# G-U-N/Phased-Consistency-Model

Measured on NVIDIA H100. Metric: distillation steps/sec (SD1.5 PCM-LoRA, bs=8/GPU), higher is better.
Workload: dtype bf16

## Files before the change

pcm_b200/csrc/gemm_epilogue.cuh:

```cuda
#pragma once
#include "gemm_params.h"

namespace pcm {

static __device__ __noinline__ void gemm_epilogue_rows_generic(const GemmParams& p, const float* sb, int m0,
                                                               int n, int r0, int cg, float* ws) {
#pragma unroll 1
  for (int i = 0; i < 2; ++i) {
    const int rr = r0 + 32 * i;
    const int m = m0 + rr;
    if (m >= p.M) continue;
    const float* srow = sb + rr * 32;
    if (ws) {
      const float4 a0 = *reinterpret_cast<const float4*>(srow + ((2 * cg) ^ (rr & 7)) * 4);
      const float4 a1 = *reinterpret_cast<const float4*>(srow + ((2 * cg + 1) ^ (rr & 7)) * 4);
      const float f[8] = {a0.x, a0.y, a0.z, a0.w, a1.x, a1.y, a1.z, a1.w};
      float* wp = ws + static_cast<long long>(m) * p.N + n;
      if (n + 8 <= p.N && (p.N & 3) == 0) {
        *reinterpret_cast<float4*>(wp) = make_float4(f[0] * p.alpha, f[1] * p.alpha, f[2] * p.alpha, f[3] * p.alpha);
        *reinterpret_cast<float4*>(wp + 4) = make_float4(f[4] * p.alpha, f[5] * p.alpha, f[6] * p.alpha, f[7] * p.alpha);
      } else {
#pragma unroll
        for (int e = 0; e < 8; ++e)
          if (n + e < p.N) wp[e] = f[e] * p.alpha;
// ... 111 lines not shown
#pragma unroll
      for (int i = 0; i < 2; ++i) {
        if (!valid[i]) continue;
        const float4 a0 = lds128(ld_a0 + i * 4096);
        const float4 a1 = lds128(ld_a1 + i * 4096);
        float f[8] = {a0.x, a0.y, a0.z, a0.w, a1.x, a1.y, a1.z, a1.w};
        if (p.alpha != 1.0f) {
#pragma unroll
          for (int e = 0; e < 8; ++e) f[e] *= p.alpha;
        }
        f[0] += bia0.x; f[1] += bia0.y; f[2] += bia0.z; f[3] += bia0.w;
        f[4] += bia1.x; f[5] += bia1.y; f[6] += bia1.z; f[7] += bia1.w;
        if (has_rv) add_bf16x8(f, rrv[i]);
        if (has_res) add_bf16x8(f, rcur[i]);
        uint4 u;
        u.x = pack_bf16x2(f[0], f[1]);
        u.y = pack_bf16x2(f[2], f[3]);
        u.z = pack_bf16x2(f[4], f[5]);
        u.w = pack_bf16x2(f[6], f[7]);
        *reinterpret_cast<uint4*>(reinterpret_cast<bf16*>(p.out) + off[i] + n) = u;
      }
      if (has_res) {
#pragma unroll
        for (int i = 0; i < 2; ++i) rcur[i] = rnext[i];
        load_res(rnext, j + 2);
      }
    } else if (n < p.N) {
      gemm_epilogue_rows_generic(p, sb, m0, n, r0, cg, ws);
    }
    asm volatile("bar.sync %0, 128;" ::"r"(bar) : "memory");
  }
}

}
```

pcm_b200/csrc/gemm_params.h:

```cpp
#pragma once
#include <cuda.h>
#include "common.cuh"
#include "../../include/pcm_b200.h"

namespace pcm {

struct KEntry {
  int a_map, b_map, dw, dh, nchunks, a_c0, b_k0;
  unsigned short n_lo, n_hi;
  int m_hi;
  int kend;
};

struct alignas(64) GemmParams {
  CUtensorMap a_maps[PCM_MAX_ASRC];
  CUtensorMap b_maps[PCM_MAX_BSRC];
  KEntry prog[PCM_MAX_PROG];
  int num_prog, lin;
  int M, N;
  int geoW, geoHW;
  int block_n, tiles_m, tiles_n, num_kblocks, num_stages;
  void* out;
  const float* bias;
  const bf16* rowvec;
  const bf16* residual;
  long long osW, osH, osB, rowvec_ld;
  int epiW, epiHW;
  int out_fp32, round_bf16;
  float alpha;
  int act;
  int b_blocked;
  int dep_a_map;
  int filtered;
  int ksplit;
  float* ws;
};

constexpr int kATileBytes = 128 * 128;

}
```

pcm_b200/csrc/gemm_tc.cu:

```cuda
#include "common.cuh"
#include "wgmma.cuh"
#include "host_common.h"
#include "../../include/pcm_b200.h"
#include "gemm_params.h"
#include "gemm_epilogue.cuh"

namespace pcm {

constexpr int kGemmThreads = 384;
constexpr int kWgradThreads = 256;
constexpr int kMaxStages = 8;
constexpr int kStagingBytes = 2 * 64 * 32 * 4;
constexpr int kSmemLimit = 227 * 1024 - 512;

__device__ __forceinline__ int tile_kblocks(const GemmParams& p, int m0, int n0) {
  int nkb = 0;
  for (int e = 0; e < p.num_prog; ++e) {
    const KEntry en = p.prog[e];
    if ((en.n_hi == 0 || (n0 >= en.n_lo && n0 < en.n_hi)) && (en.m_hi == 0 || m0 < en.m_hi))
      nkb += en.nchunks;
  }
  return nkb;
}

__device__ __forceinline__ int chunk_ksteps(int kend, int c) {
  const int w = kend - 64 * c;
  return w >= 64 ? 4 : (w <= 16 ? 1 : (w + 15) >> 4);
}

template <int BN, bool NARROW>
__global__ void __launch_bounds__(kGemmThreads, 1)
pcm_gemm_kernel(const __grid_constant__ GemmParams p) {
  extern __shared__ uint8_t smem_raw[];
  uint8_t* smem = reinterpret_cast<uint8_t*>((reinterpret_cast<uintptr_t>(smem_raw) + 1023) &
                                             ~static_cast<uintptr_t>(1023));
  __shared__ __align__(8) uint64_t full_bar[kMaxStages];
  __shared__ __align__(8) uint64_t empty_bar[kMaxStages];
  __shared__ int stage_ksteps[NARROW ? kMaxStages : 1];

  const int wg = threadIdx.x >> 7;
  const int S = p.num_stages;
  constexpr uint32_t stage_bytes = kATileBytes + BN * 128;
  const int num_items = p.tiles_m * p.tiles_n * p.ksplit;
  const int kb_per = (p.num_kblocks + p.ksplit - 1) / p.ksplit;

  if (threadIdx.x == 0) {
    for (int i = 0; i < PCM_MAX_ASRC; ++i) tma_prefetch_desc(&p.a_maps[i]);
    for (int i = 0; i < PCM_MAX_BSRC; ++i) tma_prefetch_desc(&p.b_maps[i]);
    for (int i = 0; i < S; ++i) {
      mbar_init(&full_bar[i], 1);
      mbar_init(&empty_bar[i], 2);
    }
    fence_barrier_init();
  }
  __syncthreads();
  if (p.dep_a_map < 0) griddep_sync();
  else griddep_launch();

  if (wg == 0) {
    regs_dealloc<40>();
    if (threadIdx.x == 0) {
      int stage = 0;
      uint32_t phase = 0;
      bool dep_waited = p.dep_a_map < 0;
      for (int item = blockIdx.x; item < num_items; item += gridDim.x) {
        const int tile = item / p.ksplit, ks = item - tile * p.ksplit;
        const int kb0 = ks * kb_per, kb1 = min(p.num_kblocks, kb0 + kb_per);
        int tm = tile / p.tiles_n;
        const int tn = tile - tm * p.tiles_n;
        if (p.dep_a_map >= 0) tm = p.tiles_m - 1 - tm;
        const int m0 = tm * 128, n0 = tn * BN;
        int b0 = 0, h0 = 0;
        if (!p.lin) {
          b0 = m0 / p.geoHW;
          h0 = (m0 - b0 * p.geoHW) / p.geoW;
        }
        int kidx = 0;
        for (int e = 0; e < p.num_prog; ++e) {
          const KEntry en = p.prog[e];
          if (en.n_hi != 0 && (n0 < en.n_lo || n0 >= en.n_hi)) continue;
          if (en.m_hi != 0 && m0 >= en.m_hi) continue;
          if (kidx + en.nchunks <= kb0 || kidx >= kb1) {
            kidx += en.nchunks;
            continue;
          }
          if (!dep_waited && en.a_map == p.dep_a_map) {
            griddep_wait();
            dep_waited = true;
          }
          for (int c = 0; c < en.nchunks; ++c, ++kidx) {
            if (kidx < kb0 || kidx >= kb1) continue;
            mbar_wait(&empty_bar[stage], phase ^ 1);
            if constexpr (NARROW) stage_ksteps[stage] = chunk_ksteps(en.kend, c);
            mbar_arrive_expect_tx(&full_bar[stage], stage_bytes);
            uint8_t* sa = smem + stage * stage_bytes;
            uint8_t* sb = sa + kATileBytes;
            if (p.lin)
              tma_load_4d(sa, &p.a_maps[en.a_map], &full_bar[stage], en.a_c0 + c * 64, m0, 0, 0);
            else
              tma_load_4d(sa, &p.a_maps[en.a_map], &full_bar[stage], en.a_c0 + c * 64, en.dw,
                          h0 + en.dh, b0);
            if ((p.b_blocked >> en.b_map) & 1)
              tma_load_3d(sb, &p.b_maps[en.b_map], &full_bar[stage], 0, n0, (en.b_k0 >> 6) + c);
            else
              tma_load_2d(sb, &p.b_maps[en.b_map], &full_bar[stage], en.b_k0 + c * 64, n0);
            if (++stage == S) {
              stage = 0;
              phase ^= 1;
            }
          }
        }
      }
    }
  } else {
    regs_alloc<232>();
    const int cw = wg - 1;
    const int et = threadIdx.x & 127;
    float* sbuf = reinterpret_cast<float*>(smem + S * stage_bytes) + cw * (64 * 32);
    float acc[BN / 2];
    int stage = 0;
    uint32_t phase = 0;
    for (int item = blockIdx.x; item < num_items; item += gridDim.x) {
      const int tile = item / p.ksplit, ks = item - tile * p.ksplit;
      int tm = tile / p.tiles_n;
      const int tn = tile - tm * p.tiles_n;
      if (p.dep_a_map >= 0) tm = p.tiles_m - 1 - tm;
      const int n0 = tn * BN;
      const int nkb = p.filtered ? tile_kblocks(p, tm * 128, n0)
                                 : min(p.num_kblocks, (ks + 1) * kb_per) - ks * kb_per;
      if (nkb <= 0) {
#pragma unroll
        for (int i = 0; i < BN / 2; ++i) acc[i] = 0.f;
      }
      int prev_stage = -1;
      for (int kb = 0; kb < nkb; ++kb) {
        mbar_wait(&full_bar[stage], phase);
        const uint32_t a_addr = smem_u32(smem + stage * stage_bytes) + cw * (64 * 128);
        const uint32_t b_addr = smem_u32(smem + stage * stage_bytes) + kATileBytes;
        wgmma_fence();
        if constexpr (NARROW) {
          const int nk = stage_ksteps[stage];
#pragma unroll
          for (int k = 0; k < 4; ++k)
            if (k < nk)
              Wgmma<BN, 0, 0>::mma(acc, wgmma_desc_sw128(a_addr + k * 32, 16, 1024),
                                   wgmma_desc_sw128(b_addr + k * 32, 16, 1024), (kb | k) != 0 ? 1u : 0u);
        } else {
#pragma unroll
          for (int k = 0; k < 4; ++k)
            Wgmma<BN, 0, 0>::mma(acc, wgmma_desc_sw128(a_addr + k * 32, 16, 1024),
                                 wgmma_desc_sw128(b_addr + k * 32, 16, 1024), (kb | k) != 0 ? 1u : 0u);
        }
        wgmma_commit();
        wgmma_fence_acc(acc);
        wgmma_wait<1>();
        if (prev_stage >= 0 && et == 0) mbar_arrive(&empty_bar[prev_stage]);
        prev_stage = stage;
        if (++stage == S) {
          stage = 0;
          phase ^= 1;
        }
      }
      wgmma_wait<0>();
      wgmma_fence_acc(acc);
      if (prev_stage >= 0 && et == 0) mbar_arrive(&empty_bar[prev_stage]);
      float* ws = p.ws ? p.ws + static_cast<long long>(ks) * p.M * p.N : nullptr;
      gemm_epilogue_tile<BN>(p, tm * 128 + cw * 64, n0, acc, sbuf, et, 1 + cw, ws);
    }
  }
}

__global__ void splitk_finalize_kernel(const GemmParams p) {
  griddep_sync();
  const int nvec = (p.N + 7) >> 3;
  const long long total = static_cast<long long>(p.M) * nvec;
  const long long slice = static_cast<long long>(p.M) * p.N;
  const bool vec = (p.N & 7) == 0;
  for (long long v = blockIdx.x * static_cast<long long>(blockDim.x) + threadIdx.x; v < total;
       v += static_cast<long long>(gridDim.x) * blockDim.x) {
    const int m = static_cast<int>(v / nvec);
    const int n = static_cast<int>(v - static_cast<long long>(m) * nvec) * 8;
    const int b = m / p.epiHW;
    const int r = m - b * p.epiHW;
    const int h = r / p.epiW;
    const int w = r - h * p.epiW;
    const long long o = b * p.osB + h * p.osH + w * p.osW;
    float x[8];
    const float* wp = p.ws + static_cast<long long>(m) * p.N + n;
    if (vec) {
      float4 a0 = *reinterpret_cast<const float4*>(wp), a1 = *reinterpret_cast<const float4*>(wp + 4);
#pragma unroll 4
      for (int k = 1; k < p.ksplit; ++k) {
        const float4 b0 = *reinterpret_cast<const float4*>(wp + k * slice);
        const float4 b1 = *reinterpret_cast<const float4*>(wp + k * slice + 4);
        a0.x += b0.x; a0.y += b0.y; a0.z += b0.z; a0.w += b0.w;
        a1.x += b1.x; a1.y += b1.y; a1.z += b1.z; a1.w += b1.w;
      }
      x[0] = a0.x; x[1] = a0.y; x[2] = a0.z; x[3] = a0.w;
      x[4] = a1.x; x[5] = a1.y; x[6] = a1.z; x[7] = a1.w;
    } else {
// ... 169 lines not shown
        atomicExch(sem, blockIdx.z + 1 == gridDim.z ? 0 : static_cast<int>(blockIdx.z) + 1);
    }
  }
}

static int encode_asrc(CUtensorMap* map, const pcm_asrc& a, int lin, int geoW, int geoH,
                       int box_c = 64) {
  cuuint64_t dims[4];
  cuuint64_t strides[3];
  cuuint32_t box[4];
  cuuint32_t estr[4] = {1, 1, 1, 1};
  if (lin) {
    dims[0] = a.C; dims[1] = a.W; dims[2] = 1; dims[3] = 1;
    strides[0] = a.sW * 2;
    strides[1] = static_cast<cuuint64_t>(a.sW) * 2 * a.W;
    strides[2] = strides[1];
    box[0] = box_c; box[1] = 128; box[2] = 1; box[3] = 1;
  } else {
    dims[0] = a.C; dims[1] = a.W; dims[2] = a.H; dims[3] = a.B;
    strides[0] = a.sW * 2; strides[1] = a.sH * 2; strides[2] = a.sB * 2;
    const int bw = geoW;
    if (bw > 128 || 128 % bw != 0) return set_error("conv geometry: W must divide 128");
    int bh = 128 / bw;
    if (bh > geoH) bh = geoH;
    int bb = 128 / (bw * bh);
    if (bw * bh * bb != 128) return set_error("conv geometry: H*W must divide or be divisible by 128");
    box[0] = box_c; box[1] = bw; box[2] = bh; box[3] = bb;
  }
  return encode_tmap(map, a.ptr, 4, dims, strides, box, estr);
}

typedef void (*GemmKernel)(const GemmParams);
template <bool NARROW>
static GemmKernel gemm_kernel_for(int block_n) {
  switch (block_n) {
    case 32: return pcm_gemm_kernel<32, NARROW>;
    case 64: return pcm_gemm_kernel<64, NARROW>;
    case 96: return pcm_gemm_kernel<96, NARROW>;
    case 128: return pcm_gemm_kernel<128, NARROW>;
    case 160: return pcm_gemm_kernel<160, NARROW>;
    case 192: return pcm_gemm_kernel<192, NARROW>;
    case 224: return pcm_gemm_kernel<224, NARROW>;
    default: return pcm_gemm_kernel<256, NARROW>;
  }
}

static bool misaligned(const void* p, uintptr_t a) { return (reinterpret_cast<uintptr_t>(p) & (a - 1)) != 0; }

static bool gemm_ranged(const pcm_gemm_desc* d) {
  for (int e = 0; e < d->num_prog; ++e)
    if (d->prog[e].n_hi != 0) return true;
  return false;
}

static int gemm_ksplit(const pcm_gemm_desc* d) {
  if (d->ksplit <= 1 || d->splitk_ws == nullptr || gemm_ranged(d)) return 1;
  int nkb = 0;
  for (int e = 0; e < d->num_prog; ++e) nkb += d->prog[e].nchunks;
  if (nkb < 1) return 1;
  const int ks = d->ksplit < nkb ? d->ksplit : nkb;
  const int per = (nkb + ks - 1) / ks;
  return (nkb + per - 1) / per;
}

static int validate_gemm(const pcm_gemm_desc* d) {
  if (d->block_n < 32 || d->block_n > 256 || (d->block_n % 32) != 0)
    return set_error("pcm_gemm: block_n must be a multiple of 32 in [32, 256]");
  if (d->num_a < 1 || d->num_a > PCM_MAX_ASRC || d->num_b < 1 || d->num_b > PCM_MAX_BSRC ||
      d->num_prog < 1 || d->num_prog > PCM_MAX_PROG)
    return set_error("pcm_gemm: bad source / program counts");
  if (d->M < 1) return set_error("pcm_gemm: M must be >= 1");
  if (d->N < 1) return set_error("pcm_gemm: N must be >= 1");
  if (d->out == nullptr) return set_error("pcm_gemm: out is null");
  if (!d->lin && (d->geoW < 1 || d->geoH < 1)) return set_error("pcm_gemm: geoW and geoH must be >= 1 in conv mode");
  if (!d->lin && d->epiW < 1) return set_error("pcm_gemm: epiW must be >= 1 in conv mode");
  if (!d->lin && d->epiHW < 1) return set_error("pcm_gemm: epiHW must be >= 1 in conv mode");
  if (d->act != 0 && d->act != 1) return set_error("pcm_gemm: act must be 0 or 1");
  if (d->dep_a_src1 < 0 || d->dep_a_src1 > d->num_a) return set_error("pcm_gemm: bad dep_a_src1");
  if (d->ksplit > 1 && !gemm_ranged(d)) {
    if (d->splitk_ws == nullptr) return set_error("pcm_gemm: ksplit > 1 needs splitk_ws");
    if (misaligned(d->splitk_ws, 16)) return set_error("pcm_gemm: splitk_ws is not 16-byte aligned");
  }
  const bool wide = !d->out_fp32 && d->act == 0 && gemm_ksplit(d) == 1;
  const bool vec = wide && d->N >= 32;
  const bool vec_res = wide && d->residual != nullptr && d->N >= 8;
  if (misaligned(d->out, vec ? 16 : (d->out_fp32 ? 4 : 2)))
    return set_error(vec ? "pcm_gemm: out is not 16-byte aligned" : "pcm_gemm: out is not aligned to its element size");
  if (d->bias && misaligned(d->bias, vec ? 16 : 4))
    return set_error(vec ? "pcm_gemm: bias is not 16-byte aligned" : "pcm_gemm: bias is not 4-byte aligned");
  if (d->rowvec && misaligned(d->rowvec, vec ? 16 : 2))
    return set_error(vec ? "pcm_gemm: rowvec is not 16-byte aligned" : "pcm_gemm: rowvec is not 2-byte aligned");
  if (d->residual && misaligned(d->residual, vec_res ? 16 : 2))
    return set_error(vec_res ? "pcm_gemm: residual is not 16-byte aligned" : "pcm_gemm: residual is not 2-byte aligned");
  if (vec || vec_res) {
    if (d->osW % 8 != 0) return set_error("pcm_gemm: osW is not a multiple of 8");
    if (d->osH % 8 != 0) return set_error("pcm_gemm: osH is not a multiple of 8");
    if (d->osB % 8 != 0) return set_error("pcm_gemm: osB is not a multiple of 8");
  }
  if (vec && d->rowvec && d->rowvec_ld % 8 != 0) return set_error("pcm_gemm: rowvec_ld is not a multiple of 8");
  return 0;
}

static int validate_wgrad(const pcm_wgrad_desc* d) {
  if (d->M < 1) return set_error("pcm_wgrad: M must be >= 1");
  if (d->out == nullptr) return set_error("pcm_wgrad: out is null");
  if (d->os_row == 0) return set_error("pcm_wgrad: os_row is zero");
  if (d->os_col == 0) return set_error("pcm_wgrad: os_col is zero");
  if (d->num_taps < 1 || d->num_taps > 9) return set_error("pcm_wgrad: bad tap count");
  if (!d->lin && (d->geoW < 1 || d->geoH < 1)) return set_error("pcm_wgrad: geoW and geoH must be >= 1 in conv mode");
  const int qw = d->q.C - d->q_c0 < 64 ? d->q.C - d->q_c0 : 64;
  if (d->q_c0 < 0 || qw < 8 || qw % 8 != 0)
    return set_error("pcm_wgrad: the rank slice q[:, q_c0:] must hold a positive multiple of 8 columns");
  const bool pairs = d->os_col == 1;
  if (misaligned(d->out, pairs ? 8 : 4))
    return set_error(pairs ? "pcm_wgrad: out is not 8-byte aligned" : "pcm_wgrad: out is not 4-byte aligned");
  if (pairs && d->os_row % 2 != 0) return set_error("pcm_wgrad: os_row is odd with os_col == 1");
  for (int t = 0; pairs && t < d->num_taps; ++t)
    if (d->tap_off[t] % 2 != 0) return set_error("pcm_wgrad: tap_off is odd with os_col == 1");
  if (d->sem && misaligned(d->sem, 4)) return set_error("pcm_wgrad: sem is not 4-byte aligned");
  return 0;
}

static int launch_gemm(const pcm_gemm_desc* d, cudaStream_t stream) {
  if (int rc = validate_gemm(d)) return rc;
  static GemmParams p;
  memset(&p, 0, sizeof(p));
  for (int i = 0; i < PCM_MAX_ASRC; ++i) {
    const pcm_asrc& a = d->a[i < d->num_a ? i : 0];
    if (int rc = encode_asrc(&p.a_maps[i], a, d->lin, d->geoW, d->geoH)) return rc;
  }
  for (int i = 0; i < PCM_MAX_BSRC; ++i) {
    const pcm_bsrc& b = d->b[i < d->num_b ? i : 0];
    if (b.kblocked) {
      if (b.K % 64 != 0) return set_error("pcm_gemm: K-blocked B source needs K % 64 == 0");
      cuuint64_t dims[3] = {64, static_cast<cuuint64_t>(b.N), static_cast<cuuint64_t>(b.K / 64)};
      cuuint64_t strides[2] = {128, static_cast<cuuint64_t>(b.N) * 128};
      cuuint32_t box[3] = {64, static_cast<cuuint32_t>(d->block_n), 1};
      cuuint32_t estr[3] = {1, 1, 1};
      if (int rc = encode_tmap(&p.b_maps[i], b.ptr, 3, dims, strides, box, estr)) return rc;
      if (i < d->num_b) p.b_blocked |= 1 << i;
    } else {
      cuuint64_t dims[2] = {static_cast<cuuint64_t>(b.K), static_cast<cuuint64_t>(b.N)};
      cuuint64_t strides[1] = {static_cast<cuuint64_t>(b.ld) * 2};
      cuuint32_t box[2] = {64, static_cast<cuuint32_t>(d->block_n)};
      cuuint32_t estr[2] = {1, 1};
      if (int rc = encode_tmap(&p.b_maps[i], b.ptr, 2, dims, strides, box, estr)) return rc;
    }
  }
  int nkb = 0;
  bool narrow = false;
  for (int e = 0; e < d->num_prog; ++e) {
    const pcm_kentry& k = d->prog[e];
    if (k.a_src < 0 || k.a_src >= d->num_a || k.b_src < 0 || k.b_src >= d->num_b || k.nchunks < 1 ||
        k.a_c0 < 0 || k.b_k0 < 0 || (k.b_k0 & (d->b[k.b_src].kblocked ? 63 : 7)) != 0)
      return set_error("pcm_gemm: bad K program entry");
    const int a_left = d->a[k.a_src].C - k.a_c0, b_left = d->b[k.b_src].K - k.b_k0;
    const int kend = a_left < b_left ? a_left : b_left;
    if (kend < 64 * k.nchunks) narrow = true;
    p.prog[e] = KEntry{k.a_src, k.b_src, k.dw, k.dh, k.nchunks, k.a_c0, k.b_k0, k.n_lo, k.n_hi, 0, kend};
    {
      const pcm_asrc& a = d->a[k.a_src];
      const long long rows = d->lin ? a.W : static_cast<long long>(a.B) * d->geoW * d->geoH;
      if (rows < d->M && rows % 128 == 0 && d->ksplit <= 1) {
        p.prog[e].m_hi = static_cast<int>(rows);
        p.filtered = 1;
      }
    }
    nkb += k.nchunks;
    if (k.n_hi != 0) {
      if (k.n_lo % d->block_n != 0 || (k.n_hi % d->block_n != 0 && k.n_hi < d->N) || k.n_hi <= k.n_lo)
        return set_error("pcm_gemm: K entry N range must be aligned to block_n");
      p.filtered = 1;
    }
  }
  p.num_prog = d->num_prog;
  p.lin = d->lin;
  p.M = d->M;
  p.N = d->N;
  p.geoW = d->lin ? 1 : d->geoW;
  p.geoHW = d->lin ? 1 : d->geoW * d->geoH;
  p.block_n = d->block_n;
  p.tiles_m = (d->M + 127) / 128;
  p.tiles_n = (d->N + d->block_n - 1) / d->block_n;
  p.num_kblocks = nkb;
  const int stage_bytes = kATileBytes + d->block_n * 128;
  int S = (kSmemLimit - 1024 - kStagingBytes) / stage_bytes;
  if (S > kMaxStages) S = kMaxStages;
  if (S < 2) return set_error("pcm_gemm: tile too large for shared memory");
  p.num_stages = S;
  p.out = d->out;
  p.bias = d->bias;
  p.rowvec = reinterpret_cast<const bf16*>(d->rowvec);
  p.residual = reinterpret_cast<const bf16*>(d->residual);
  p.osW = d->osW; p.osH = d->osH; p.osB = d->osB;
  p.rowvec_ld = d->rowvec_ld;
  p.epiW = d->epiW > 0 ? d->epiW : 1;
  p.epiHW = d->epiHW > 0 ? d->epiHW : 1;
  p.out_fp32 = d->out_fp32;
  p.round_bf16 = d->round_bf16;
  p.alpha = d->alpha;
  p.act = d->act;
  p.ws = nullptr;
  p.dep_a_map = -1;
  p.ksplit = gemm_ksplit(d);

  const size_t smem = static_cast<size_t>(S) * stage_bytes + kStagingBytes + 1024;
  const GemmKernel kernel = narrow ? gemm_kernel_for<true>(d->block_n) : gemm_kernel_for<false>(d->block_n);
  static bool attr_set[2][9] = {};
  if (!attr_set[narrow][d->block_n / 32]) {
    CUDA_TRY(cudaFuncSetAttribute(kernel, cudaFuncAttributeMaxDynamicSharedMemorySize, kSmemLimit));
    attr_set[narrow][d->block_n / 32] = true;
  }
  if (d->dep_a_src1 > 0 && p.ksplit == 1) {
    p.dep_a_map = d->dep_a_src1 - 1;
  }
  const int tiles = p.tiles_m * p.tiles_n * p.ksplit;
  const int grid = tiles < num_sms() ? tiles : num_sms();
  if (p.ksplit > 1) {
    GemmParams q = p;
    q.ws = reinterpret_cast<float*>(d->splitk_ws);
    q.bias = nullptr; q.rowvec = nullptr; q.residual = nullptr; q.act = 0;
    CUDA_TRY(launch_pdl(kernel, dim3(grid), dim3(kGemmThreads), smem, stream, q));
    GemmParams f = p;
    f.ws = q.ws;
    f.alpha = 1.f;
    const long long nv = static_cast<long long>(p.M) * ((p.N + 7) / 8);
    int fg = static_cast<int>((nv + 255) / 256);
    if (fg > num_sms() * 8) fg = num_sms() * 8;
    CUDA_TRY(launch_pdl(splitk_finalize_kernel, dim3(fg), dim3(256), 0, stream, f));
    return 0;
  }
  CUDA_TRY(launch_pdl(kernel, dim3(grid), dim3(kGemmThreads), smem, stream, p));
  CUDA_TRY(cudaGetLastError());
  return 0;
}

static int launch_wgrad(const pcm_wgrad_desc* d, cudaStream_t stream) {
  if (int rc = validate_wgrad(d)) return rc;
  static WgradParams p;
  memset(&p, 0, sizeof(p));
  if (int rc = encode_asrc(&p.p_map, d->p, d->lin, d->geoW, d->geoH)) return rc;
  if (int rc = encode_asrc(&p.q_map, d->q, d->lin, d->geoW, d->geoH)) return rc;
  p.lin = d->lin;
  p.geoW = d->lin ? 1 : d->geoW;
// ... 17 lines not shown
    if (ks > max_ks) ks = max_ks;
    if (ks < 1) ks = 1;
  }
  if (ks > p.kblocks_total) ks = p.kblocks_total;
  {
    const int per = (p.kblocks_total + ks - 1) / ks;
    ks = (p.kblocks_total + per - 1) / per;
  }
  p.ksplit = ks;
  p.sem = reinterpret_cast<int*>(d->sem);
  p.out = d->out;
  p.os_row = d->os_row;
  p.os_col = d->os_col;
  p.alpha = d->alpha;
  const size_t smem = static_cast<size_t>(kWgStages) * kWgStageBytes + 1024;
  static bool attr_set = false;
  if (!attr_set) {
    CUDA_TRY(cudaFuncSetAttribute(pcm_wgrad_kernel, cudaFuncAttributeMaxDynamicSharedMemorySize,
                                  220 * 1024));
    attr_set = true;
  }
  dim3 grid(ch_tiles, d->num_taps, ks);
  CUDA_TRY(launch_pdl(pcm_wgrad_kernel, dim3(grid), dim3(kWgradThreads), smem, stream, p));
  CUDA_TRY(cudaGetLastError());
  return 0;
}

}

extern "C" int pcm_gemm(const pcm_gemm_desc* d, void* stream) {
  return pcm::launch_gemm(d, reinterpret_cast<cudaStream_t>(stream));
}
extern "C" int pcm_gemm_check(const pcm_gemm_desc* d) { return pcm::validate_gemm(d); }
extern "C" int pcm_wgrad_check(const pcm_wgrad_desc* d) { return pcm::validate_wgrad(d); }
extern "C" int pcm_wgrad(const pcm_wgrad_desc* d, void* stream) {
  return pcm::launch_wgrad(d, reinterpret_cast<cudaStream_t>(stream));
}
```

include/pcm_b200.h:

```cpp
#ifndef PCM_B200_H
#define PCM_B200_H
#include <stdint.h>

#ifdef __cplusplus
extern "C" {
#endif

#define PCM_MAX_ASRC 6
#define PCM_MAX_BSRC 4
#define PCM_MAX_PROG 24

typedef struct {
  const void* ptr;
  int32_t C, W, H, B;
  int64_t sW, sH, sB;
} pcm_asrc;

typedef struct {
  const void* ptr;
  int32_t K, N;
  int64_t ld;
  int32_t kblocked;
} pcm_bsrc;

// ... 20 lines not shown
  int32_t epiW, epiHW;
  int32_t out_fp32, round_bf16;
  float alpha;
  int32_t act;
  int32_t ksplit;
  void* splitk_ws;
  int32_t dep_a_src1;
} pcm_gemm_desc;

typedef struct {
  pcm_asrc p;
  pcm_asrc q;
  int32_t q_c0;
  int32_t lin;
  int32_t M;
  int32_t geoW, geoH;
  int32_t num_taps;
  int32_t dw[9], dh[9];
  int64_t tap_off[9];
  float* out;
  int64_t os_row, os_col;
  int32_t ksplit;
  float alpha;
  void* sem;
} pcm_wgrad_desc;

const char* pcm_last_error(void);
int pcm_version(void);
int pcm_num_sms(void);

int pcm_gemm(const pcm_gemm_desc* d, void* stream);
int pcm_wgrad(const pcm_wgrad_desc* d, void* stream);
int pcm_gemm_check(const pcm_gemm_desc* d);
int pcm_wgrad_check(const pcm_wgrad_desc* d);

int64_t pcm_groupnorm_ws_bytes(int B, int HW, int C, int G);
int pcm_groupnorm_fwd(const void* x1, const void* x2, int C1, int C2, int B, int HW, int G,
                      const float* gamma, const float* beta, float eps, int silu, void* out,
                      float* stats, void* ws, int64_t ws_bytes, void* stream);
int pcm_groupnorm_fwd_part(const void* x1, const void* x2, int C1, int C2, int B, int part_B, int HW,
                           int G, const float* gamma, const float* beta, float eps, int silu, void* out,
                           float* stats, void* ws, int64_t ws_bytes, void* stream);
int pcm_groupnorm_bwd(const void* dy, const void* x1, const void* x2, int C1, int C2, int B, int HW,
                      int G, const float* gamma, const float* beta, float eps, int silu,
                      const float* stats, float* red, const void* add, void* dx1, void* dx2,
                      float* colsum ,
                      void* ws, int64_t ws_bytes, void* stream);
int pcm_layernorm_fwd(const void* x, int M, int C, const float* gamma, const float* beta, float eps,
                      void* out, float* stats, void* stream);
int pcm_layernorm_bwd(const void* dy, const void* x, int M, int C, const float* gamma,
                      const float* stats, const void* add, void* dx, void* stream);

int pcm_attn_fwd(const void* q, const void* k, const void* v, void* out, float* lse, int B, int H,
                 int Sq, int Skv, int D, int64_t ldq, int64_t ldk, int64_t ldv, int64_t ldo,
                 float scale, void* stream);
int pcm_attn_bwd(const void* q, const void* k, const void* v, const void* o, const void* dout,
                 const float* lse, float* delta, void* dq, void* dk, void* dv, int B, int H, int Sq,
                 int Skv, int D, int64_t ldq, int64_t ldk, int64_t ldv, int64_t ldo, float scale,
                 void* stream);

int pcm_geglu_fwd(const void* u, int64_t M, int F, void* out, void* stream);
int pcm_geglu_bwd(const void* dgg, const void* u, int64_t M, int F, void* du, void* stream);
int pcm_upsample2x_fwd(const void* in, int B, int H, int W, int C, void* out, void* stream);
int pcm_upsample2x_bwd(const void* dout, int B, int H, int W, int C, void* din, void* stream);
int pcm_conv3x3_c4(const float* in, int B, int H, int W, int C, const void* w, const float* bias,
                   int sgn, int round_in, void* out, void* stream);
// ... 47 lines not shown
```

pcm_b200/_lib.py:

```python
import ctypes as C
import os

_HERE = os.path.dirname(os.path.abspath(__file__))
LIB_PATH = os.environ.get("PCM_B200_LIB") or os.path.join(_HERE, "lib", "libpcm_b200.so")

MAX_ASRC, MAX_BSRC, MAX_PROG = 6, 4, 24
SUMSQ_WS_DOUBLES = 1024


class ASrc(C.Structure):
    _fields_ = [("ptr", C.c_void_p), ("C", C.c_int32), ("W", C.c_int32), ("H", C.c_int32),
                ("B", C.c_int32), ("sW", C.c_int64), ("sH", C.c_int64), ("sB", C.c_int64)]


class BSrc(C.Structure):
    _fields_ = [("ptr", C.c_void_p), ("K", C.c_int32), ("N", C.c_int32), ("ld", C.c_int64), ("kblocked", C.c_int32)]


class KEntry(C.Structure):
    _fields_ = [("a_src", C.c_int32), ("b_src", C.c_int32), ("dw", C.c_int32), ("dh", C.c_int32),
                ("nchunks", C.c_int32), ("a_c0", C.c_int32), ("b_k0", C.c_int32), ("n_lo", C.c_uint16), ("n_hi", C.c_uint16)]


class GemmDesc(C.Structure):
# ... 22 lines not shown

_lib = None


def lib():
    global _lib
    if _lib is None:
        if not os.path.exists(LIB_PATH):
            raise RuntimeError(
                f"{LIB_PATH} is missing: the pcm_b200 CUDA extension is not built. "
                "Run `python -c \"import __graft_entry__ as g; g.build()\"` (needs nvcc). "
                "There is no CPU fallback for the product path.")
        _lib = C.CDLL(LIB_PATH)
        _lib.pcm_last_error.restype = C.c_char_p
        for name in EXPORTS:
            fn = getattr(_lib, name)
            if name == "pcm_groupnorm_ws_bytes":
                fn.restype = C.c_int64
            elif name not in ("pcm_last_error",):
                fn.restype = C.c_int
            if name in ARGTYPES:
                fn.argtypes = ARGTYPES[name]
    return _lib


EXPORTS = [
    "pcm_last_error",
    "pcm_version",
    "pcm_num_sms",
    "pcm_gemm",
    "pcm_wgrad",
    "pcm_gemm_check",
    "pcm_wgrad_check",
    "pcm_groupnorm_ws_bytes",
    "pcm_groupnorm_fwd",
    "pcm_groupnorm_fwd_part",
    "pcm_groupnorm_bwd",
    "pcm_layernorm_fwd",
    "pcm_layernorm_bwd",
    "pcm_attn_fwd",
    "pcm_attn_bwd",
    "pcm_geglu_fwd",
    "pcm_geglu_bwd",
    "pcm_upsample2x_fwd",
    "pcm_upsample2x_bwd",
    "pcm_conv3x3_c4",
    "pcm_timestep_embed",
    "pcm_colsum",
    "pcm_add_bf16",
    "pcm_cast_f32_bf16",
    "pcm_prepare",
    "pcm_add_noise",
    "pcm_teacher_step",
    "pcm_teacher_substep",
    "pcm_loss",
    "pcm_noise_travel",
    "pcm_axpby_f64",
    "pcm_fm_step",
    "pcm_grad_sumsq",
    "pcm_adamw_clip",
    "pcm_ema_update",
    "pcm_lora_refresh",
    "pcm_lora_fuse",
    "pcm_sample_step",
]


P, I, L64, F, D = C.c_void_p, C.c_int, C.c_int64, C.c_float, C.c_double
ARGTYPES = {
    "pcm_gemm": [P, P],
    "pcm_wgrad": [P, P],
    "pcm_gemm_check": [P],
    "pcm_wgrad_check": [P],
    "pcm_groupnorm_ws_bytes": [I, I, I, I],
    "pcm_groupnorm_fwd": [P, P, I, I, I, I, I, P, P, F, I, P, P, P, L64, P],
    "pcm_groupnorm_fwd_part": [P, P, I, I, I, I, I, I, P, P, F, I, P, P, P, L64, P],
    "pcm_groupnorm_bwd": [P, P, P, I, I, I, I, I, P, P, F, I, P, P, P, P, P, P, P, L64, P],
    "pcm_layernorm_fwd": [P, I, I, P, P, F, P, P, P],
    "pcm_layernorm_bwd": [P, P, I, I, P, P, P, P, P],
    "pcm_attn_fwd": [P, P, P, P, P, I, I, I, I, I, L64, L64, L64, L64, F, P],
    "pcm_attn_bwd": [P, P, P, P, P, P, P, P, P, P, I, I, I, I, I, L64, L64, L64, L64, F, P],
    "pcm_geglu_fwd": [P, L64, I, P, P],
    "pcm_geglu_bwd": [P, P, L64, I, P, P],
    "pcm_upsample2x_fwd": [P, I, I, I, I, P, P],
    "pcm_upsample2x_bwd": [P, I, I, I, I, P, P],
    "pcm_conv3x3_c4": [P, I, I, I, I, P, P, I, I, P, P],
    "pcm_timestep_embed": [P, I, I, P, P],
    "pcm_colsum": [P, I, I, I, P, P],
    "pcm_add_bf16": [P, P, L64, P, P],
    "pcm_cast_f32_bf16": [P, L64, P, P],
    "pcm_prepare": [P, I, I, P, I, P, P, I, I, P, P, P, P, P],
    "pcm_add_noise": [P, P, P, L64, I, I, P, P],
    "pcm_teacher_step": [P, P, P, P, L64, I, I, P, P],
    "pcm_teacher_substep": [P, P, P, P, P, P, P, L64, I, I, P, P],
    "pcm_loss": [P, P, P, P, P, L64, I, I, F, I, P, P, P, P, P],
    "pcm_noise_travel": [P, P, P, P, P, L64, I, P, P],
    "pcm_axpby_f64": [P, P, P, P, L64, I, P, P],
    "pcm_fm_step": [P, P, P, P, P, L64, I, I, P, P],
    "pcm_grad_sumsq": [P, L64, P, P],
    "pcm_adamw_clip": [P, P, P, P, L64, P, F, F, F, F, F, F, P, I, P],
    "pcm_ema_update": [P, P, L64, F, P],
    "pcm_lora_refresh": [P, P, I, L64, F, P, P],
    "pcm_lora_fuse": [P, P, I, L64, F, P],
    "pcm_sample_step": [P, P, P, P, L64, I, I, P, D, D, D, D, I, P],
}

# ... 9 lines not shown
```

Measured before the change: 8.828.

## Add TMA-based GEMM epilogue with residual prefetch and overlapped stores

Adds a TMA epilogue path for the persistent wgmma GEMM. Consumers write the bf16 result into a swizzled shared-memory tile. The producer warp then issues TMA stores for that tile while the next tile's mainloop continues, and it can TMA-prefetch the residual tile into the same buffer ahead of time. This replaces per-thread global stores and residual loads with bulk async transfers and overlaps them with compute. In exchange it adds mbarrier handshakes between producer and consumers, and the epilogue buffer grows, which can reduce the number of pipeline stages for wide tiles.

```diff
diff --git a/pcm_b200/csrc/gemm_epilogue.cuh b/pcm_b200/csrc/gemm_epilogue.cuh
--- a/pcm_b200/csrc/gemm_epilogue.cuh
+++ b/pcm_b200/csrc/gemm_epilogue.cuh
@@ -167,4 +167,72 @@
   }
 }
 
-}
+
+template <int W>
+__device__ __forceinline__ uint32_t epi_tile_offset(int r, int g, int et) {
+  constexpr int kFull = W / 64;
+  if (g < 8 * kFull) return (g >> 3) * (128 * 128) + r * 128 + (((g & 7) ^ (r & 7)) << 4) + 4 * (et & 3);
+  return kFull * (128 * 128) + r * 64 + (((g & 3) ^ ((r >> 1) & 3)) << 4) + 4 * (et & 3);
+}
+
+template <int BN, int W, int SL>
+__device__ __forceinline__ void gemm_epilogue_tile_smem(const GemmParams& p, int m0, int n0, int cw,
+                                                        const float (&acc)[BN / 2], uint32_t buf, int et) {
+  const bool has_bias = p.bias != nullptr, has_rv = p.rowvec != nullptr, has_res = p.residual != nullptr;
+  const int r = cw * 64 + ((et >> 5) << 4) + ((et & 31) >> 2);
+  const bf16* rvp[2] = {nullptr, nullptr};
+#pragma unroll
+  for (int i = 0; i < 2; ++i) {
+    const int m = m0 + r + 8 * i;
+    if (has_rv && m < p.M) rvp[i] = p.rowvec + static_cast<long long>(m / p.epiHW) * p.rowvec_ld;
+  }
+  const int c = 2 * (et & 3);
+#pragma unroll
+  for (int gs = 0; gs < W / 8; ++gs) {
+    const int g = SL * (W / 8) + gs;
+    const int n = n0 + 8 * g + c;
+    float2 bia = make_float2(0.f, 0.f);
+    if (has_bias) bia = *reinterpret_cast<const float2*>(p.bias + n);
+#pragma unroll
+    for (int i = 0; i < 2; ++i) {
+      const uint32_t addr = buf + epi_tile_offset<W>(r + 8 * i, gs, et);
+      float x0 = acc[4 * g + 2 * i], x1 = acc[4 * g + 2 * i + 1];
+      if (p.alpha != 1.0f) {
+        x0 = __fmul_rn(x0, p.alpha);
+        x1 = __fmul_rn(x1, p.alpha);
+      }
+      x0 = __fadd_rn(x0, bia.x);
+      x1 = __fadd_rn(x1, bia.y);
+      if (rvp[i]) {
+        const float2 t = unpack_bf16x2(*reinterpret_cast<const uint32_t*>(rvp[i] + n));
+        x0 = __fadd_rn(x0, t.x);
+        x1 = __fadd_rn(x1, t.y);
+      }
+      if (has_res) {
+        uint32_t u;
+        asm volatile("ld.shared.b32 %0, [%1];" : "=r"(u) : "r"(addr) : "memory");
+        const float2 t = unpack_bf16x2(u);
+        x0 = __fadd_rn(x0, t.x);
+        x1 = __fadd_rn(x1, t.y);
+      }
+      asm volatile("st.shared.b32 [%0], %1;" ::"r"(addr), "r"(pack_bf16x2(x0, x1)) : "memory");
+    }
+  }
+}
+
+template <int W, bool STORE>
+__device__ __forceinline__ void gemm_epilogue_tma(const GemmParams& p, uint8_t* buf, uint64_t* bar, int m0, int n0) {
+  const int b = m0 / p.epiHW, rem = m0 - b * p.epiHW, h = rem / p.epiW, w = rem - h * p.epiW;
+  constexpr int kFull = W / 64;
+#pragma unroll
+  for (int j = 0; j <= kFull; ++j) {
+    if (j == kFull && W % 64 == 0) break;
+    const int t = j < kFull ? 0 : 1;
+    if constexpr (STORE)
+      tma_store_4d(&p.out_maps[t], smem_u32(buf + j * (128 * 128)), n0 + 64 * j, w, h, b);
+    else
+      tma_load_4d(buf + j * (128 * 128), &p.res_maps[t], bar, n0 + 64 * j, w, h, b);
+  }
+}
+
+}
diff --git a/pcm_b200/csrc/gemm_params.h b/pcm_b200/csrc/gemm_params.h
--- a/pcm_b200/csrc/gemm_params.h
+++ b/pcm_b200/csrc/gemm_params.h
@@ -34,7 +34,12 @@
   int filtered;
   int ksplit;
   float* ws;
+  CUtensorMap out_maps[2];
+  CUtensorMap res_maps[2];
+  int tma_epi;
 };
+
+__host__ __device__ constexpr int tma_epi_cols(int bn) { return bn <= 160 ? bn : (bn == 256 ? 128 : 0); }
 
 constexpr int kATileBytes = 128 * 128;
 
diff --git a/pcm_b200/csrc/gemm_tc.cu b/pcm_b200/csrc/gemm_tc.cu
--- a/pcm_b200/csrc/gemm_tc.cu
+++ b/pcm_b200/csrc/gemm_tc.cu
@@ -37,12 +37,17 @@
   __shared__ __align__(8) uint64_t full_bar[kMaxStages];
   __shared__ __align__(8) uint64_t empty_bar[kMaxStages];
   __shared__ int stage_ksteps[NARROW ? kMaxStages : 1];
+  __shared__ __align__(8) uint64_t buf_full, epi_done;
+  constexpr int kEpiW = tma_epi_cols(BN);
+  constexpr bool kTmaEpi = kEpiW > 0;
+  constexpr int kSlices = kTmaEpi ? BN / kEpiW : 1;
 
   const int wg = threadIdx.x >> 7;
   const int S = p.num_stages;
   constexpr uint32_t stage_bytes = kATileBytes + BN * 128;
   const int num_items = p.tiles_m * p.tiles_n * p.ksplit;
   const int kb_per = (p.num_kblocks + p.ksplit - 1) / p.ksplit;
+  uint8_t* ebuf = smem + S * stage_bytes;
 
   if (threadIdx.x == 0) {
     for (int i = 0; i < PCM_MAX_ASRC; ++i) tma_prefetch_desc(&p.a_maps[i]);
@@ -51,6 +56,10 @@
       mbar_init(&full_bar[i], 1);
       mbar_init(&empty_bar[i], 2);
     }
+    if constexpr (kTmaEpi) {
+      mbar_init(&buf_full, 1);
+      mbar_init(&epi_done, 2);
+    }
     fence_barrier_init();
   }
   __syncthreads();
@@ -63,6 +72,43 @@
       int stage = 0;
       uint32_t phase = 0;
       bool dep_waited = p.dep_a_map < 0;
+      bool have_prev = false, prev_tma = false;
+      int prev_m0 = 0, prev_n0 = 0;
+      uint32_t epi_phase = 0;
+      auto store_prev = [&](bool last) {
+        for (int sl = 0; sl < kSlices; ++sl) {
+          mbar_wait(&epi_done, epi_phase);
+          epi_phase ^= 1;
+          if (prev_tma) {
+            gemm_epilogue_tma<kEpiW, true>(p, ebuf, nullptr, prev_m0, prev_n0 + sl * kEpiW);
+            tma_store_commit();
+          }
+          if (sl + 1 < kSlices || !last) {
+            if (prev_tma) tma_store_wait_read<0>();
+            if (sl + 1 < kSlices) mbar_arrive(&buf_full);
+          }
+        }
+      };
+      auto hand_over = [&](int m0, int n0) {
+        if (have_prev) store_prev(false);
+        const bool tma = p.tma_epi && n0 + BN <= p.N;
+        if (kSlices == 1 && tma && p.residual) {
+          mbar_arrive_expect_tx(&buf_full, 128 * BN * 2);
+          gemm_epilogue_tma<kEpiW, false>(p, ebuf, &buf_full, m0, n0);
+        } else {
+          mbar_arrive(&buf_full);
+        }
+        have_prev = true;
+        prev_tma = tma;
+        prev_m0 = m0;
+        prev_n0 = n0;
+      };
+      if (kTmaEpi && p.tma_epi) {
+        for (int i = 0; i < 2; ++i) {
+          tma_prefetch_desc(&p.out_maps[i]);
+          tma_prefetch_desc(&p.res_maps[i]);
+        }
+      }
       for (int item = blockIdx.x; item < num_items; item += gridDim.x) {
         const int tile = item / p.ksplit, ks = item - tile * p.ksplit;
         const int kb0 = ks * kb_per, kb1 = min(p.num_kblocks, kb0 + kb_per);
@@ -70,6 +116,8 @@
         const int tn = tile - tm * p.tiles_n;
         if (p.dep_a_map >= 0) tm = p.tiles_m - 1 - tm;
         const int m0 = tm * 128, n0 = tn * BN;
+        int issued = 0;
+        bool handed = !(kTmaEpi && p.tma_epi);
         int b0 = 0, h0 = 0;
         if (!p.lin) {
           b0 = m0 / p.geoHW;
@@ -108,18 +156,28 @@
               stage = 0;
               phase ^= 1;
             }
+            if (!handed && ++issued == S) {
+              hand_over(m0, n0);
+              handed = true;
+            }
           }
         }
+        if (!handed) hand_over(m0, n0);
+      }
+      if (kTmaEpi && p.tma_epi) {
+        if (have_prev) store_prev(true);
+        tma_store_wait_all();
       }
     }
   } else {
     regs_alloc<232>();
     const int cw = wg - 1;
     const int et = threadIdx.x & 127;
-    float* sbuf = reinterpret_cast<float*>(smem + S * stage_bytes) + cw * (64 * 32);
+    float* sbuf = reinterpret_cast<float*>(ebuf) + cw * (64 * 32);
     float acc[BN / 2];
     int stage = 0;
     uint32_t phase = 0;
+    uint32_t buf_phase = 0;
     for (int item = blockIdx.x; item < num_items; item += gridDim.x) {
       const int tile = item / p.ksplit, ks = item - tile * p.ksplit;
       int tm = tile / p.tiles_n;
@@ -165,7 +223,25 @@
       wgmma_fence_acc(acc);
       if (prev_stage >= 0 && et == 0) mbar_arrive(&empty_bar[prev_stage]);
       float* ws = p.ws ? p.ws + static_cast<long long>(ks) * p.M * p.N : nullptr;
-      gemm_epilogue_tile<BN>(p, tm * 128 + cw * 64, n0, acc, sbuf, et, 1 + cw, ws);
+      if (kTmaEpi && p.tma_epi) {
+        const bool tma = p.tma_epi && n0 + BN <= p.N;
+#pragma unroll
+        for (int sl = 0; sl < kSlices; ++sl) {
+          mbar_wait(&buf_full, buf_phase);
+          buf_phase ^= 1;
+          if (tma) {
+            if (sl == 0) gemm_epilogue_tile_smem<BN, kEpiW, 0>(p, tm * 128, n0, cw, acc, smem_u32(ebuf), et);
+            else gemm_epilogue_tile_smem<BN, kEpiW, kSlices - 1>(p, tm * 128, n0, cw, acc, smem_u32(ebuf), et);
+          } else if (sl == 0) {
+            gemm_epilogue_tile<BN>(p, tm * 128 + cw * 64, n0, acc, sbuf, et, 1 + cw, ws);
+          }
+          fence_proxy_async();
+          asm volatile("bar.sync %0, 128;" ::"r"(1 + cw) : "memory");
+          if (et == 0) mbar_arrive(&epi_done);
+        }
+      } else {
+        gemm_epilogue_tile<BN>(p, tm * 128 + cw * 64, n0, acc, sbuf, et, 1 + cw, ws);
+      }
     }
   }
 }
@@ -490,6 +566,48 @@
   return 0;
 }
 
+static int gemm_epi_bytes(int block_n) {
+  return tma_epi_cols(block_n) * 256 > kStagingBytes ? tma_epi_cols(block_n) * 256 : kStagingBytes;
+}
+
+static int encode_epilogue_maps(const pcm_gemm_desc* d, GemmParams* p) {
+  p->tma_epi = 0;
+  if (tma_epi_cols(d->block_n) == 0 || d->out_fp32 || d->act != 0 || p->ksplit != 1 || d->N < d->block_n) return 0;
+  if (tma_epi_cols(d->block_n) < d->block_n && d->residual) return 0;
+  if (p->tiles_m * p->tiles_n <= num_sms()) return 0;
+  cuuint64_t dims[4], strides[3];
+  cuuint32_t box[4];
+  cuuint32_t estr[4] = {1, 1, 1, 1};
+  const long long row = d->osW * 2;
+  if (p->epiW >= d->M) {
+    dims[1] = d->M; dims[2] = 1; dims[3] = 1;
+    strides[0] = row; strides[1] = row * d->M; strides[2] = strides[1];
+    box[1] = 128; box[2] = 1; box[3] = 1;
+  } else {
+    const int W = p->epiW, HW = p->epiHW;
+    if (HW % W != 0 || d->M % HW != 0 || W > 128 || 128 % W != 0 || (HW % 128 != 0 && 128 % HW != 0)) return 0;
+    const int H = HW / W;
+    const int bh = 128 / W < H ? 128 / W : H;
+    dims[1] = W; dims[2] = H; dims[3] = d->M / HW;
+    strides[0] = row; strides[1] = d->osH * 2; strides[2] = d->osB * 2;
+    if (H == 1) strides[1] = row * W;
+    if (dims[3] == 1) strides[2] = strides[1] * H;
+    box[1] = W; box[2] = bh; box[3] = 128 / (W * bh);
+  }
+  dims[0] = d->N;
+  for (int i = 0; i < 3; ++i)
+    if (strides[i] == 0 || strides[i] % 16 != 0 || strides[i] >= (1ll << 40)) return 0;
+  for (int t = 0; t < 2; ++t) {
+    box[0] = t == 0 ? 64 : 32;
+    const int swz = t == 0 ? 128 : 64;
+    if (int rc = encode_tmap(&p->out_maps[t], d->out, 4, dims, strides, box, estr, swz)) return rc;
+    if (d->residual)
+      if (int rc = encode_tmap(&p->res_maps[t], d->residual, 4, dims, strides, box, estr, swz)) return rc;
+  }
+  p->tma_epi = 1;
+  return 0;
+}
+
 static int launch_gemm(const pcm_gemm_desc* d, cudaStream_t stream) {
   if (int rc = validate_gemm(d)) return rc;
   static GemmParams p;
@@ -553,7 +671,8 @@
   p.tiles_n = (d->N + d->block_n - 1) / d->block_n;
   p.num_kblocks = nkb;
   const int stage_bytes = kATileBytes + d->block_n * 128;
-  int S = (kSmemLimit - 1024 - kStagingBytes) / stage_bytes;
+  const int epi_bytes = gemm_epi_bytes(d->block_n);
+  int S = (kSmemLimit - 1024 - epi_bytes) / stage_bytes;
   if (S > kMaxStages) S = kMaxStages;
   if (S < 2) return set_error("pcm_gemm: tile too large for shared memory");
   p.num_stages = S;
@@ -572,8 +691,9 @@
   p.ws = nullptr;
   p.dep_a_map = -1;
   p.ksplit = gemm_ksplit(d);
-
-  const size_t smem = static_cast<size_t>(S) * stage_bytes + kStagingBytes + 1024;
+  if (int rc = encode_epilogue_maps(d, &p)) return rc;
+
+  const size_t smem = static_cast<size_t>(S) * stage_bytes + epi_bytes + 1024;
   const GemmKernel kernel = narrow ? gemm_kernel_for<true>(d->block_n) : gemm_kernel_for<false>(d->block_n);
   static bool attr_set[2][9] = {};
   if (!attr_set[narrow][d->block_n / 32]) {
```

Result: faster. 9.094 (median of 6 runs) (+3.0%).

## Add 256-row GEMM tiles for long-K GEMMs with block_n 128/160

Applied to the files above, without the earlier changes.

Templates the warp-specialized GEMM kernel on an M-subtile count so each consumer warpgroup computes two 64-row subtiles against one shared B tile. The producer issues two A TMA loads per stage. A host-side planner picks 256-row tiles only when block_n is 128 or 160, there is no split-K, K is long enough, and the wave count does not get worse. The aim is to halve B-tile traffic per output and improve wgmma issue efficiency. The cost is larger stages (fewer pipeline stages), higher register pressure (240 regs for consumers, 24 for the producer) and coarser tiles.

```diff
diff --git a/include/pcm_b200.h b/include/pcm_b200.h
--- a/include/pcm_b200.h
+++ b/include/pcm_b200.h
@@ -76,6 +76,7 @@
 int pcm_gemm(const pcm_gemm_desc* d, void* stream);
 int pcm_wgrad(const pcm_wgrad_desc* d, void* stream);
 int pcm_gemm_check(const pcm_gemm_desc* d);
+int pcm_gemm_plan_rows(const pcm_gemm_desc* d);
 int pcm_wgrad_check(const pcm_wgrad_desc* d);
 
 int64_t pcm_groupnorm_ws_bytes(int B, int HW, int C, int G);
diff --git a/pcm_b200/_lib.py b/pcm_b200/_lib.py
--- a/pcm_b200/_lib.py
+++ b/pcm_b200/_lib.py
@@ -78,6 +78,7 @@
     "pcm_wgrad",
     "pcm_gemm_check",
     "pcm_wgrad_check",
+    "pcm_gemm_plan_rows",
     "pcm_groupnorm_ws_bytes",
     "pcm_groupnorm_fwd",
     "pcm_groupnorm_fwd_part",
@@ -118,6 +119,7 @@
     "pcm_wgrad": [P, P],
     "pcm_gemm_check": [P],
     "pcm_wgrad_check": [P],
+    "pcm_gemm_plan_rows": [P],
     "pcm_groupnorm_ws_bytes": [I, I, I, I],
     "pcm_groupnorm_fwd": [P, P, I, I, I, I, I, P, P, F, I, P, P, P, L64, P],
     "pcm_groupnorm_fwd_part": [P, P, I, I, I, I, I, I, P, P, F, I, P, P, P, L64, P],
diff --git a/pcm_b200/csrc/gemm_tc.cu b/pcm_b200/csrc/gemm_tc.cu
--- a/pcm_b200/csrc/gemm_tc.cu
+++ b/pcm_b200/csrc/gemm_tc.cu
@@ -28,7 +28,7 @@
   return w >= 64 ? 4 : (w <= 16 ? 1 : (w + 15) >> 4);
 }
 
-template <int BN, bool NARROW>
+template <int BN, int MS, bool NARROW>
 __global__ void __launch_bounds__(kGemmThreads, 1)
 pcm_gemm_kernel(const __grid_constant__ GemmParams p) {
   extern __shared__ uint8_t smem_raw[];
@@ -40,7 +40,8 @@
 
   const int wg = threadIdx.x >> 7;
   const int S = p.num_stages;
-  constexpr uint32_t stage_bytes = kATileBytes + BN * 128;
+  constexpr int kRows = 128 * MS;
+  constexpr uint32_t stage_bytes = MS * kATileBytes + BN * 128;
   const int num_items = p.tiles_m * p.tiles_n * p.ksplit;
   const int kb_per = (p.num_kblocks + p.ksplit - 1) / p.ksplit;
 
@@ -58,7 +59,7 @@
   else griddep_launch();
 
   if (wg == 0) {
-    regs_dealloc<40>();
+    regs_dealloc<MS == 2 ? 24 : 40>();
     if (threadIdx.x == 0) {
       int stage = 0;
       uint32_t phase = 0;
@@ -69,11 +70,14 @@
         int tm = tile / p.tiles_n;
         const int tn = tile - tm * p.tiles_n;
         if (p.dep_a_map >= 0) tm = p.tiles_m - 1 - tm;
-        const int m0 = tm * 128, n0 = tn * BN;
-        int b0 = 0, h0 = 0;
+        const int m0 = tm * kRows, n0 = tn * BN;
+        int b0[MS] = {}, h0[MS] = {};
         if (!p.lin) {
-          b0 = m0 / p.geoHW;
-          h0 = (m0 - b0 * p.geoHW) / p.geoW;
+#pragma unroll
+          for (int s = 0; s < MS; ++s) {
+            b0[s] = (m0 + 128 * s) / p.geoHW;
+            h0[s] = (m0 + 128 * s - b0[s] * p.geoHW) / p.geoW;
+          }
         }
         int kidx = 0;
         for (int e = 0; e < p.num_prog; ++e) {
@@ -94,12 +98,16 @@
             if constexpr (NARROW) stage_ksteps[stage] = chunk_ksteps(en.kend, c);
             mbar_arrive_expect_tx(&full_bar[stage], stage_bytes);
             uint8_t* sa = smem + stage * stage_bytes;
-            uint8_t* sb = sa + kATileBytes;
-            if (p.lin)
-              tma_load_4d(sa, &p.a_maps[en.a_map], &full_bar[stage], en.a_c0 + c * 64, m0, 0, 0);
-            else
-              tma_load_4d(sa, &p.a_maps[en.a_map], &full_bar[stage], en.a_c0 + c * 64, en.dw,
-                          h0 + en.dh, b0);
+            uint8_t* sb = sa + MS * kATileBytes;
+#pragma unroll
+            for (int s = 0; s < MS; ++s) {
+              if (p.lin)
+                tma_load_4d(sa + s * kATileBytes, &p.a_maps[en.a_map], &full_bar[stage], en.a_c0 + c * 64,
+                            m0 + 128 * s, 0, 0);
+              else
+                tma_load_4d(sa + s * kATileBytes, &p.a_maps[en.a_map], &full_bar[stage], en.a_c0 + c * 64,
+                            en.dw, h0[s] + en.dh, b0[s]);
+            }
             if ((p.b_blocked >> en.b_map) & 1)
               tma_load_3d(sb, &p.b_maps[en.b_map], &full_bar[stage], 0, n0, (en.b_k0 >> 6) + c);
             else
@@ -113,11 +121,11 @@
       }
     }
   } else {
-    regs_alloc<232>();
+    regs_alloc<MS == 2 ? 240 : 232>();
     const int cw = wg - 1;
     const int et = threadIdx.x & 127;
     float* sbuf = reinterpret_cast<float*>(smem + S * stage_bytes) + cw * (64 * 32);
-    float acc[BN / 2];
+    float acc[MS][BN / 2];
     int stage = 0;
     uint32_t phase = 0;
     for (int item = blockIdx.x; item < num_items; item += gridDim.x) {
@@ -126,33 +134,40 @@
       const int tn = tile - tm * p.tiles_n;
       if (p.dep_a_map >= 0) tm = p.tiles_m - 1 - tm;
       const int n0 = tn * BN;
-      const int nkb = p.filtered ? tile_kblocks(p, tm * 128, n0)
+      const int nkb = p.filtered ? tile_kblocks(p, tm * kRows, n0)
                                  : min(p.num_kblocks, (ks + 1) * kb_per) - ks * kb_per;
       if (nkb <= 0) {
 #pragma unroll
-        for (int i = 0; i < BN / 2; ++i) acc[i] = 0.f;
+        for (int s = 0; s < MS; ++s)
+#pragma unroll
+          for (int i = 0; i < BN / 2; ++i) acc[s][i] = 0.f;
       }
       int prev_stage = -1;
       for (int kb = 0; kb < nkb; ++kb) {
         mbar_wait(&full_bar[stage], phase);
-        const uint32_t a_addr = smem_u32(smem + stage * stage_bytes) + cw * (64 * 128);
-        const uint32_t b_addr = smem_u32(smem + stage * stage_bytes) + kATileBytes;
+        const uint32_t a_addr = smem_u32(smem + stage * stage_bytes) + cw * MS * (64 * 128);
+        const uint32_t b_addr = smem_u32(smem + stage * stage_bytes) + MS * kATileBytes;
         wgmma_fence();
         if constexpr (NARROW) {
           const int nk = stage_ksteps[stage];
 #pragma unroll
           for (int k = 0; k < 4; ++k)
             if (k < nk)
-              Wgmma<BN, 0, 0>::mma(acc, wgmma_desc_sw128(a_addr + k * 32, 16, 1024),
+#pragma unroll
+              for (int s = 0; s < MS; ++s)
+                Wgmma<BN, 0, 0>::mma(acc[s], wgmma_desc_sw128(a_addr + s * (64 * 128) + k * 32, 16, 1024),
+                                     wgmma_desc_sw128(b_addr + k * 32, 16, 1024), (kb | k) != 0 ? 1u : 0u);
+        } else {
+#pragma unroll
+          for (int k = 0; k < 4; ++k)
+#pragma unroll
+            for (int s = 0; s < MS; ++s)
+              Wgmma<BN, 0, 0>::mma(acc[s], wgmma_desc_sw128(a_addr + s * (64 * 128) + k * 32, 16, 1024),
                                    wgmma_desc_sw128(b_addr + k * 32, 16, 1024), (kb | k) != 0 ? 1u : 0u);
-        } else {
-#pragma unroll
-          for (int k = 0; k < 4; ++k)
-            Wgmma<BN, 0, 0>::mma(acc, wgmma_desc_sw128(a_addr + k * 32, 16, 1024),
-                                 wgmma_desc_sw128(b_addr + k * 32, 16, 1024), (kb | k) != 0 ? 1u : 0u);
         }
         wgmma_commit();
-        wgmma_fence_acc(acc);
+#pragma unroll
+        for (int s = 0; s < MS; ++s) wgmma_fence_acc(acc[s]);
         wgmma_wait<1>();
         if (prev_stage >= 0 && et == 0) mbar_arrive(&empty_bar[prev_stage]);
         prev_stage = stage;
@@ -162,10 +177,13 @@
         }
       }
       wgmma_wait<0>();
-      wgmma_fence_acc(acc);
+#pragma unroll
+      for (int s = 0; s < MS; ++s) wgmma_fence_acc(acc[s]);
       if (prev_stage >= 0 && et == 0) mbar_arrive(&empty_bar[prev_stage]);
       float* ws = p.ws ? p.ws + static_cast<long long>(ks) * p.M * p.N : nullptr;
-      gemm_epilogue_tile<BN>(p, tm * 128 + cw * 64, n0, acc, sbuf, et, 1 + cw, ws);
+#pragma unroll
+      for (int s = 0; s < MS; ++s)
+        gemm_epilogue_tile<BN>(p, tm * kRows + (cw * MS + s) * 64, n0, acc[s], sbuf, et, 1 + cw, ws);
     }
   }
 }
@@ -401,16 +419,17 @@
 
 typedef void (*GemmKernel)(const GemmParams);
 template <bool NARROW>
-static GemmKernel gemm_kernel_for(int block_n) {
+static GemmKernel gemm_kernel_for(int block_n, int rows) {
+  if (rows == 256) return block_n == 128 ? pcm_gemm_kernel<128, 2, NARROW> : pcm_gemm_kernel<160, 2, NARROW>;
   switch (block_n) {
-    case 32: return pcm_gemm_kernel<32, NARROW>;
-    case 64: return pcm_gemm_kernel<64, NARROW>;
-    case 96: return pcm_gemm_kernel<96, NARROW>;
-    case 128: return pcm_gemm_kernel<128, NARROW>;
-    case 160: return pcm_gemm_kernel<160, NARROW>;
-    case 192: return pcm_gemm_kernel<192, NARROW>;
-    case 224: return pcm_gemm_kernel<224, NARROW>;
-    default: return pcm_gemm_kernel<256, NARROW>;
+    case 32: return pcm_gemm_kernel<32, 1, NARROW>;
+    case 64: return pcm_gemm_kernel<64, 1, NARROW>;
+    case 96: return pcm_gemm_kernel<96, 1, NARROW>;
+    case 128: return pcm_gemm_kernel<128, 1, NARROW>;
+    case 160: return pcm_gemm_kernel<160, 1, NARROW>;
+    case 192: return pcm_gemm_kernel<192, 1, NARROW>;
+    case 224: return pcm_gemm_kernel<224, 1, NARROW>;
+    default: return pcm_gemm_kernel<256, 1, NARROW>;
   }
 }
 
@@ -430,6 +449,26 @@
   const int ks = d->ksplit < nkb ? d->ksplit : nkb;
   const int per = (nkb + ks - 1) / ks;
   return (nkb + per - 1) / per;
+}
+
+static int gemm_entry_m_hi(const pcm_gemm_desc* d, const pcm_kentry& k) {
+  const pcm_asrc& a = d->a[k.a_src];
+  const long long rows = d->lin ? a.W : static_cast<long long>(a.B) * d->geoW * d->geoH;
+  return rows < d->M && rows % 128 == 0 && d->ksplit <= 1 ? static_cast<int>(rows) : 0;
+}
+
+constexpr int kTallMinKBlocks = 32;
+static int gemm_plan_rows(const pcm_gemm_desc* d) {
+  if ((d->block_n != 128 && d->block_n != 160) || gemm_ksplit(d) != 1) return 128;
+  int nkb = 0;
+  for (int e = 0; e < d->num_prog; ++e) {
+    if (gemm_entry_m_hi(d, d->prog[e]) % 256 != 0) return 128;
+    if (d->prog[e].n_hi == 0 && gemm_entry_m_hi(d, d->prog[e]) == 0) nkb += d->prog[e].nchunks;
+  }
+  if (nkb < kTallMinKBlocks) return 128;
+  const long long tn = (d->N + d->block_n - 1) / d->block_n, sms = num_sms();
+  const long long t128 = (d->M + 127) / 128 * tn, t256 = (d->M + 255) / 256 * tn;
+  return 2 * ((t256 + sms - 1) / sms) <= (t128 + sms - 1) / sms ? 256 : 128;
 }
 
 static int validate_gemm(const pcm_gemm_desc* d) {
@@ -526,15 +565,9 @@
     const int a_left = d->a[k.a_src].C - k.a_c0, b_left = d->b[k.b_src].K - k.b_k0;
     const int kend = a_left < b_left ? a_left : b_left;
     if (kend < 64 * k.nchunks) narrow = true;
-    p.prog[e] = KEntry{k.a_src, k.b_src, k.dw, k.dh, k.nchunks, k.a_c0, k.b_k0, k.n_lo, k.n_hi, 0, kend};
-    {
-      const pcm_asrc& a = d->a[k.a_src];
-      const long long rows = d->lin ? a.W : static_cast<long long>(a.B) * d->geoW * d->geoH;
-      if (rows < d->M && rows % 128 == 0 && d->ksplit <= 1) {
-        p.prog[e].m_hi = static_cast<int>(rows);
-        p.filtered = 1;
-      }
-    }
+    p.prog[e] = KEntry{k.a_src, k.b_src, k.dw, k.dh, k.nchunks, k.a_c0, k.b_k0, k.n_lo, k.n_hi,
+                       gemm_entry_m_hi(d, k), kend};
+    if (p.prog[e].m_hi != 0) p.filtered = 1;
     nkb += k.nchunks;
     if (k.n_hi != 0) {
       if (k.n_lo % d->block_n != 0 || (k.n_hi % d->block_n != 0 && k.n_hi < d->N) || k.n_hi <= k.n_lo)
@@ -549,10 +582,11 @@
   p.geoW = d->lin ? 1 : d->geoW;
   p.geoHW = d->lin ? 1 : d->geoW * d->geoH;
   p.block_n = d->block_n;
-  p.tiles_m = (d->M + 127) / 128;
+  const int rows = gemm_plan_rows(d);
+  p.tiles_m = (d->M + rows - 1) / rows;
   p.tiles_n = (d->N + d->block_n - 1) / d->block_n;
   p.num_kblocks = nkb;
-  const int stage_bytes = kATileBytes + d->block_n * 128;
+  const int stage_bytes = rows / 128 * kATileBytes + d->block_n * 128;
   int S = (kSmemLimit - 1024 - kStagingBytes) / stage_bytes;
   if (S > kMaxStages) S = kMaxStages;
   if (S < 2) return set_error("pcm_gemm: tile too large for shared memory");
@@ -574,11 +608,12 @@
   p.ksplit = gemm_ksplit(d);
 
   const size_t smem = static_cast<size_t>(S) * stage_bytes + kStagingBytes + 1024;
-  const GemmKernel kernel = narrow ? gemm_kernel_for<true>(d->block_n) : gemm_kernel_for<false>(d->block_n);
-  static bool attr_set[2][9] = {};
-  if (!attr_set[narrow][d->block_n / 32]) {
+  const GemmKernel kernel =
+      narrow ? gemm_kernel_for<true>(d->block_n, rows) : gemm_kernel_for<false>(d->block_n, rows);
+  static bool attr_set[2][2][9] = {};
+  if (!attr_set[rows / 256][narrow][d->block_n / 32]) {
     CUDA_TRY(cudaFuncSetAttribute(kernel, cudaFuncAttributeMaxDynamicSharedMemorySize, kSmemLimit));
-    attr_set[narrow][d->block_n / 32] = true;
+    attr_set[rows / 256][narrow][d->block_n / 32] = true;
   }
   if (d->dep_a_src1 > 0 && p.ksplit == 1) {
     p.dep_a_map = d->dep_a_src1 - 1;
@@ -662,6 +697,7 @@
   return pcm::launch_gemm(d, reinterpret_cast<cudaStream_t>(stream));
 }
 extern "C" int pcm_gemm_check(const pcm_gemm_desc* d) { return pcm::validate_gemm(d); }
+extern "C" int pcm_gemm_plan_rows(const pcm_gemm_desc* d) { return pcm::gemm_plan_rows(d); }
 extern "C" int pcm_wgrad_check(const pcm_wgrad_desc* d) { return pcm::validate_wgrad(d); }
 extern "C" int pcm_wgrad(const pcm_wgrad_desc* d, void* stream) {
   return pcm::launch_wgrad(d, reinterpret_cast<cudaStream_t>(stream));
```

Result: faster. 8.811 before, 9.081 after, median of 6 (+3.1%).
